# malak29/video-text-detection-system

Measured on AMD Instinct MI355X. Metric: frames/sec (detect+recognize) @720p, 1/2/4/8 MI355X; box IoU vs CPU ref, higher is better.
Workload: dtype f16

## Files before the change

### video-text-detection-system_amd/csrc/conv_halo.hip

```cpp
#include <cstdio>
#include <cstdlib>
#include "vtd_common.h"

namespace {

struct HaloParams {
    const half_t* in;
    const half_t* wgt;
    const float* bias;
    const half_t* res;
    half_t* out;
    int n, h, w, cin, cout;
    int in_hp, in_wp, in_ring, out_hp, out_wp, out_ring, res_hp, res_wp, res_ring;
    int tiles_x, tiles_y, tiles_n, relu;
    unsigned long long* stamps;
    const half_t* in2 = nullptr;
    int in2_hp = 0, in2_wp = 0, in2_c = 0, in2_ring = 0;
    int K = 0;
    int dbg;
};

template <int N>
__device__ __forceinline__ void hl_wait_vmcnt() {
    asm volatile("s_waitcnt vmcnt(%0)" ::"n"(N) : "memory");
}

template <int BN, int TW>
__global__ __launch_bounds__((BN / 64) * 256) void conv_halo_kernel(const HaloParams p) {
    constexpr int WN = BN / 64, NW = 4 * WN, NT = NW * 64, TH = 256 / TW;
    constexpr int HWD = TW + 2, HROWS = (TH + 2) * HWD, HPIECES = (HROWS + 7) / 8, HBYTES = HPIECES * 1024;
    constexpr int HPW = (HPIECES + NW - 1) / NW;
    constexpr int HPS = (HPW + 7) / 8;
    constexpr int BSTAGE = BN * 128, BPW = BN / 8 / NW;
    constexpr int EPI_ROW = BN * 4 + 16;
// ... 307 lines not shown
            if (p.res) {
#pragma unroll
                for (int e = 0; e < 4; ++e) { v0[e] += (float)rv[q][e]; v1[e] += (float)rv[q][4 + e]; }
            }
            half8 hv;
#pragma unroll
            for (int e = 0; e < 4; ++e) {
                hv[e] = (half_t)((p.relu && v0[e] < 0.f) ? 0.f : v0[e]);
                hv[4 + e] = (half_t)((p.relu && v1[e] < 0.f) ? 0.f : v1[e]);
            }
            *(half8*)(p.out + (((int64_t)img * p.out_hp + y + p.out_ring) * p.out_wp + x + p.out_ring) * p.cout + ch) = hv;
        }
    }
}

template <int TW>
int halo64_launch(const HaloParams& p, hipStream_t stream) {
    constexpr int TH = 256 / TW, HROWS = (TH + 2) * (TW + 2), HBYTES = (HROWS + 7) / 8 * 1024;
    constexpr int lds = HBYTES + 4 * 64 * 128;
    static_assert(lds >= 256 * (64 * 4 + 16) && 2 * lds <= 160 * 1024, "epilogue tile fits; two workgroups per CU");
    static bool attr_done = false;
    if (!attr_done) {
        hipError_t e = hipFuncSetAttribute((const void*)conv_halo64_kernel<TW>, hipFuncAttributeMaxDynamicSharedMemorySize, lds);
        if (e != hipSuccess) return -(int)e;
        attr_done = true;
    }
    hipLaunchKernelGGL((conv_halo64_kernel<TW>), dim3(p.n * p.tiles_y * p.tiles_x * p.tiles_n), dim3(256), lds, stream, p);
    return -(int)hipGetLastError();
}

constexpr int HS_HW = 18, HS_ROWS = 180, HS_PIECES = 23, HS_HALO_BYTES = 24 * 1024, HS_BSTAGE = 64 * 128;
constexpr int HS_LDS = HS_HALO_BYTES + 3 * HS_BSTAGE;

template <int N>
__device__ __forceinline__ void hs_wait_staged() {
    asm volatile("s_waitcnt vmcnt(%0) lgkmcnt(0)" ::"n"(N) : "memory");
}

__global__ __launch_bounds__(256, 3) void conv_halo_small_kernel(const HaloParams p) {
    constexpr int NW = 4, FN = 2, BPW = 2, HPW = 6;
    __shared__ __attribute__((aligned(16))) char smem[HS_LDS];
    char* const hb = smem;
    char* const bring = smem + HS_HALO_BYTES;

    const int nblk = gridDim.x, b = blockIdx.x;
    const int q8 = nblk >> 3, r8 = nblk & 7, xcd = b & 7;
    int tile = (xcd < r8 ? xcd * (q8 + 1) : r8 * (q8 + 1) + (xcd - r8) * q8) + (b >> 3);
    const int tn = tile % p.tiles_n;
    tile /= p.tiles_n;
    const int tx = tile % p.tiles_x;
    tile /= p.tiles_x;
    const int ty = tile % p.tiles_y;
    const int img = tile / p.tiles_y;
    const int y0 = ty * 8, x0 = tx * 16, n0 = tn * 64;

    const int tid = threadIdx.x, lane = tid & 63;
    const int w = __builtin_amdgcn_readfirstlane(tid >> 6);
    const int lrow = lane >> 3, fr = lane & 15, fq = lane >> 4;
    const int K = p.K, nchunks = p.cin >> 6;
    const bool dual = p.in2 != nullptr;

    int hoff[HPW];
#pragma unroll
    for (int k = 0; k < HPW; ++k) {
        int row = (w + k * NW) * 8 + lrow;
        row = row < HS_ROWS ? row : HS_ROWS - 1;
        const int hy = row / HS_HW, hx = row - hy * HS_HW;
        int gy = y0 - 1 + hy + p.in_ring, gx = x0 - 1 + hx + p.in_ring;
        gy = gy < p.in_hp ? gy : p.in_hp - 1;
        gx = gx < p.in_wp ? gx : p.in_wp - 1;
        hoff[k] = ((img * p.in_hp + gy) * p.in_wp + gx) * p.cin + ((lane & 7) ^ (hx & 6)) * 8;
    }
    auto issue_halo = [&](int chunk) {
#pragma unroll
        for (int k = 0; k < HPW; ++k)
            if (w + k * NW < HS_PIECES)
// ... 8 lines not shown
        }
    };
    const half_t* bsrc[BPW];
#pragma unroll
    for (int i = 0; i < BPW; ++i) {
        const int row = (i * NW + w) * 8 + lrow;
        const int chan = (row & 32) + ((row >> 2) & 3) * 8 + ((row >> 4) & 1) * 4 + (row & 3);
        bsrc[i] = p.wgt + (int64_t)(n0 + chan) * K + ((lane & 7) ^ ((row >> 1) & 7)) * 8;
    }
    auto issue_b = [&](int koff, int stage) {
#pragma unroll
        for (int i = 0; i < BPW; ++i)
            __builtin_amdgcn_global_load_lds((const VTD_AS1 void*)(bsrc[i] + koff), (VTD_AS3 void*)(bring + stage * HS_BSTAGE + (i * NW + w) * 1024), 16, 0, 0);
    };

    const int wm = w >> 1, wn = w & 1;
    const char* a_addr[3][2];
#pragma unroll
    for (int dx = 0; dx < 3; ++dx)
#pragma unroll
        for (int kk = 0; kk < 2; ++kk) a_addr[dx][kk] = hb + (wm * 4 * HS_HW + fr + dx) * 128 + (((fq + 4 * kk) ^ ((fr + dx) & 6)) << 4);
    const char* b_addr[2];
#pragma unroll
    for (int kk = 0; kk < 2; ++kk) b_addr[kk] = bring + (wn * FN * 16 + fr) * 128 + (((fq + 4 * kk) ^ ((fr >> 1) & 7)) << 4);
    floatx4 acc[FN][4];
#pragma unroll
    for (int i = 0; i < FN; ++i)
#pragma unroll
        for (int j = 0; j < 4; ++j) acc[i][j] = floatx4{0.f, 0.f, 0.f, 0.f};

    issue_halo(0);
    issue_b(0, 0);
    issue_b(p.cin, 1);
    for (int chunk = 0; chunk < nchunks; ++chunk) {
        const bool more = chunk + 1 < nchunks;
#pragma unroll
        for (int tap = 0; tap < 9; ++tap) {
            if (tap < 8 || more || dual) hs_wait_staged<BPW>(); else hs_wait_staged<0>();
            __builtin_amdgcn_s_barrier();
            const int tap2 = (tap + 2) % 9;
            const int koff2 = (tap == 7 && !more) ? 9 * p.cin : tap2 * p.cin + (chunk + (tap + 2 >= 9 ? 1 : 0)) * 64;
            if (tap < 7 || (tap == 7 && (more || dual))) issue_b(koff2, (tap + 2) % 3);
            const int row_off = ((tap / 3) * HS_HW) * 128, stage_off = (tap % 3) * HS_BSTAGE;
#pragma unroll
            for (int kk = 0; kk < 2; ++kk) {
                half8 af[4], bf[FN];
#pragma unroll
                for (int j = 0; j < 4; ++j) af[j] = *(const half8*)(a_addr[tap % 3][kk] + row_off + j * (HS_HW * 128));
#pragma unroll
                for (int i = 0; i < FN; ++i) bf[i] = *(const half8*)(b_addr[kk] + stage_off + i * 2048);
#pragma unroll
                for (int i = 0; i < FN; ++i)
#pragma unroll
                    for (int j = 0; j < 4; ++j) acc[i][j] = __builtin_amdgcn_mfma_f32_16x16x32_f16(bf[i], af[j], acc[i][j], 0, 0, 0);
            }
            if (tap == 8 && more) {
                asm volatile("s_waitcnt lgkmcnt(0)" ::: "memory");
                __builtin_amdgcn_s_barrier();
                issue_halo(chunk + 1);
                issue_b(koff2, (tap + 2) % 3);
            } else if (tap == 8 && dual) {
                asm volatile("s_waitcnt lgkmcnt(0)" ::: "memory");
                __builtin_amdgcn_s_barrier();
                issue_dual();
            }
        }
    }
    if (dual) {
        hs_wait_staged<0>();
        __builtin_amdgcn_s_barrier();
#pragma unroll
        for (int kk = 0; kk < 2; ++kk) {
            half8 af[4], bf[FN];
            const char* a2 = hb + (wm * 64 + fr) * 128 + (((fq + 4 * kk) ^ (fr & 6)) << 4);
#pragma unroll
            for (int j = 0; j < 4; ++j) af[j] = *(const half8*)(a2 + j * 2048);
#pragma unroll
            for (int i = 0; i < FN; ++i) bf[i] = *(const half8*)(b_addr[kk] + i * 2048);
#pragma unroll
            for (int i = 0; i < FN; ++i)
#pragma unroll
                for (int j = 0; j < 4; ++j) acc[i][j] = __builtin_amdgcn_mfma_f32_16x16x32_f16(bf[i], af[j], acc[i][j], 0, 0, 0);
        }
    }

    const int ch = n0 + wn * 32 + fq * 8;
    const floatx4 bias0 = *(const floatx4*)(p.bias + ch), bias1 = *(const floatx4*)(p.bias + ch + 4);
    const int x = x0 + fr;
    half8 rv[4];
    if (p.res) {
#pragma unroll
        for (int j = 0; j < 4; ++j) {
            int y = y0 + wm * 4 + j;
            y = y < p.h ? y : p.h - 1;
            const int xc = x < p.w ? x : p.w - 1;
            rv[j] = *(const half8*)(p.res + (((int64_t)img * p.res_hp + y + p.res_ring) * p.res_wp + xc + p.res_ring) * p.cout + ch);
        }
    }
#pragma unroll
    for (int j = 0; j < 4; ++j) {
        const int y = y0 + wm * 4 + j;
        if (y >= p.h || x >= p.w) continue;
        floatx4 v0 = acc[0][j] + bias0, v1 = acc[1][j] + bias1;
        if (p.res) {
#pragma unroll
            for (int e = 0; e < 4; ++e) { v0[e] += (float)rv[j][e]; v1[e] += (float)rv[j][4 + e]; }
        }
        half8 hv;
#pragma unroll
        for (int e = 0; e < 4; ++e) {
            hv[e] = (half_t)((p.relu && v0[e] < 0.f) ? 0.f : v0[e]);
            hv[4 + e] = (half_t)((p.relu && v1[e] < 0.f) ? 0.f : v1[e]);
        }
        *(half8*)(p.out + (((int64_t)img * p.out_hp + y + p.out_ring) * p.out_wp + x + p.out_ring) * p.cout + ch) = hv;
    }
}

template <int TW, bool RELU, bool RES>
__global__ __launch_bounds__(256, 1) void conv3x3_c64_persistent_kernel(const HaloParams p) {
    constexpr int TH = 256 / TW, HWD = TW + 2, HROWS = (TH + 2) * HWD, HPIECES = (HROWS + 7) / 8, HBYTES = HPIECES * 1024;
    constexpr int HPW = (HPIECES + 3) / 4;
    constexpr int WBYTES = 9 * 64 * 128;
    extern __shared__ __attribute__((aligned(16))) char smem[];
    char* const wl = smem;
    char* const hbuf = smem + WBYTES;

    const int tid = threadIdx.x, lane = tid & 63;
    const int w = __builtin_amdgcn_readfirstlane(tid >> 6);
    const int lrow = lane >> 3, fr = lane & 15, fq = lane >> 4;
    const int tiles_per_img = p.tiles_x * p.tiles_y, total = p.n * tiles_per_img;

#pragma unroll
    for (int k = 0; k < 18; ++k) {
        const int piece = w + 4 * k, tap = piece >> 3, row = (piece & 7) * 8 + lrow;
        const int c_log = (lane & 7) ^ ((row >> 1) & 7);
        const int cout = 16 * ((row & 15) >> 2) + 4 * (row >> 4) + (row & 3);
        __builtin_amdgcn_global_load_lds((const VTD_AS1 void*)(p.wgt + cout * 576 + tap * 64 + c_log * 8),
                                         (VTD_AS3 void*)(wl + piece * 1024), 16, 0, 0);
    }
    floatx4 bias4[4];
#pragma unroll
    for (int i = 0; i < 4; ++i) bias4[i] = *(const floatx4*)(p.bias + fq * 16 + i * 4);
#pragma unroll
    for (int i = 0; i < 4; ++i) asm volatile("" : "+v"(bias4[i]));

    auto tile_coords = [&](int t, int& img, int& y0, int& x0) {
        img = t / tiles_per_img;
        const int r = t - img * tiles_per_img, ty = r / p.tiles_x;
// ... 423 lines not shown
    p.relu = (c.flags & EPI_RELU) ? 1 : 0;
    p.stamps = nullptr;
    p.dbg = 0;
    if (c.in_y0 != c.in_x0 || c.in_y0 < 0 || c.K != 9 * c.in_c || c.out_c != c.cout || p.n <= 0 || (c.in_c & 63) || (c.cout & 63) ||
        (tw != 16 && tw != 32) || c.stride != 1 || c.M != p.n * c.ho * c.wo)
        return -2201;
    if ((int64_t)p.n * c.in_hp * c.in_wp * c.in_c >= (1ll << 31)) return -2202;
    const int th = 256 / tw;
    p.tiles_x = (p.w + tw - 1) / tw; p.tiles_y = (p.h + th - 1) / th; p.tiles_n = bn > 1 ? p.cout / bn : 1;
    if (bn == 2) {
        p.tiles_n = p.cout / 64;
        return tw == 16 ? halo64_launch<16>(p, stream) : halo64_launch<32>(p, stream);
    }
    if (bn == 1) {
        if (p.cin != 64 || p.cout != 64) return -2201;
        p.tiles_n = 1;
        return tw == 16 ? c64_dispatch<16>(p, stream) : c64_dispatch<32>(p, stream);
    }
    if (bn == 64 && tw == 16) return halo_launch<64, 16>(p, stream);
    if (bn == 64 && tw == 32) return halo_launch<64, 32>(p, stream);
    if (bn == 128 && tw == 16) return halo_launch<128, 16>(p, stream);
    if (bn == 128 && tw == 32) return halo_launch<128, 32>(p, stream);
    return -2201;
}

bool vtd_conv_halo_small_supported(const ConvParams& c) {
    if (!halo_common_rules(c, true) || c.ho % 8 || c.wo % 16) return false;
    if (c.in2 && (c.in2_mul != 2 || c.in2_shr != 0 || c.cin_steps2 != 1 || c.kw2 != 1 || c.seg1_steps * 64 != 9 * c.in_c || c.in2_c < 64 || (c.in2_c & 7) ||
                  c.in2_ring < 0 || 2 * (c.ho - 1) + c.in2_ring >= c.in2_hp || 2 * (c.wo - 1) + c.in2_ring >= c.in2_wp))
        return false;
    return c.in_hp >= c.ho + c.in_y0 + 2 && c.in_wp >= c.wo + c.in_y0 + 2;
}

int vtd_launch_conv_halo_small(const ConvParams& c, hipStream_t stream) {
    if (c.ho <= 0 || c.wo <= 0) return -2201;
    HaloParams p;
    p.in = c.in; p.wgt = c.wgt; p.bias = c.bias; p.res = (c.flags & EPI_RESIDUAL) ? c.res : nullptr; p.out = (half_t*)c.out;
    p.h = c.ho; p.w = c.wo; p.n = c.M / (c.ho * c.wo); p.cin = c.in_c; p.cout = c.cout;
    p.in_hp = c.in_hp; p.in_wp = c.in_wp; p.in_ring = c.in_y0 + 1;
    p.out_hp = c.out_hp; p.out_wp = c.out_wp; p.out_ring = c.out_ring;
    p.res_hp = c.res_hp; p.res_wp = c.res_wp; p.res_ring = c.res_ring;
    p.relu = (c.flags & EPI_RELU) ? 1 : 0;
    p.stamps = nullptr;
    p.dbg = 0;
    p.K = c.K;
    if (c.in2) { p.in2 = c.in2; p.in2_hp = c.in2_hp; p.in2_wp = c.in2_wp; p.in2_c = c.in2_c; p.in2_ring = c.in2_ring; }
    if (c.in_y0 != c.in_x0 || c.in_y0 < 0 || c.K != 9 * c.in_c + (c.in2 ? 64 : 0) || c.out_c != c.cout || p.n <= 0 || (c.in_c & 63) || (c.cout & 63) ||
        c.stride != 1 || c.M != p.n * c.ho * c.wo || (c.ho & 7) || (c.wo & 15) || ((c.flags & EPI_RESIDUAL) && !c.res) || c.plist)
        return -2201;
    if (c.in2 && (c.in2_mul != 2 || c.in2_shr != 0 || c.in2_c < 64 || (c.in2_c & 7) || c.in2_ring < 0 || 2 * (c.ho - 1) + c.in2_ring >= c.in2_hp ||
                  2 * (c.wo - 1) + c.in2_ring >= c.in2_wp || (int64_t)p.n * c.in2_hp * c.in2_wp * c.in2_c >= (1ll << 31)))
        return -2201;
    if (c.in_hp < c.ho + p.in_ring + 1 || c.in_wp < c.wo + p.in_ring + 1 || c.out_ring < 0 || c.out_hp < c.ho + c.out_ring || c.out_wp < c.wo + c.out_ring ||
        (p.res && (c.res_ring < 0 || c.res_hp < c.ho + c.res_ring || c.res_wp < c.wo + c.res_ring)))
        return -2201;
    if ((int64_t)p.n * c.in_hp * c.in_wp * c.in_c >= (1ll << 31)) return -2202;
    p.tiles_x = p.w / 16; p.tiles_y = p.h / 8; p.tiles_n = p.cout / 64;
    hipLaunchKernelGGL(conv_halo_small_kernel, dim3(p.n * p.tiles_y * p.tiles_x * p.tiles_n), dim3(256), 0, stream, p);
    return -(int)hipGetLastError();
}
```

### video-text-detection-system_amd/csrc/vtd_api.cpp

```cpp
#include <algorithm>
#include <cmath>
#include <cstdio>
#include <cstdlib>
#include <cstring>
#include <map>
#include <memory>
#include <string>
#include <vector>

#include "../../include/vtd.h"
#include "vtd_common.h"

int vtd_launch_conv(const ConvParams& p, int cfg, hipStream_t stream);
int vtd_conv_num_configs();
bool vtd_conv_config_valid(const ConvParams& p, int cfg);
int vtd_launch_preprocess(const uint8_t* frames, int n, int H, int W, half_t* out, const int* xb, const int* xk, int ksx,
                          const int* yb, const int* yk, int ksy, int max_rows, hipStream_t stream);
int vtd_launch_nchw_to_input(const float* x, half_t* out, int n, hipStream_t stream);
int vtd_launch_maxpool(const TensorDesc& in, const TensorDesc& out, int n, int kh, int kw, int sh, int sw, int pad_h, int pad_w,
                       hipStream_t stream);
void vtd_stem_pool_pack_weights(const float* w_folded, half_t* packed);
int vtd_launch_stem_pool(const TensorDesc& in, const TensorDesc& out, const half_t* w_packed, const float* bias, int n, hipStream_t stream);
extern "C" int vtd_head_entry_halo_steps(int py, int px, int nch1, int* out);
int vtd_launch_head_entry_halo(const ConvParams& c, const int* steps_dev, int nsteps, int big_tiles, hipStream_t stream);
#ifdef VTD_EXPERIMENTAL_CANDIDATES
extern "C" int vtd_head_entry_half_schedule(const int* steps, int nsteps, int* out);
int vtd_launch_head_entry_half(const ConvParams& c, const int* sched_dev, int nsteps, hipStream_t stream);
int vtd_head_entry_pair_tables(int py, int px, int c2ch, int* half_steps, int* plan);
int vtd_launch_head_entry_pair(const ConvParams& c, const int* half_steps_dev, const int* plan_dev, int nh, hipStream_t stream);
#endif
bool vtd_conv_halo_supported(const ConvParams& c, int* bn_out, int* tw_out);
bool vtd_conv_halo_c64_supported(const ConvParams& c, int tw);
int vtd_launch_conv_halo(const ConvParams& c, int bn, int tw, hipStream_t stream);
bool vtd_conv_halo_small_supported(const ConvParams& c);
int vtd_launch_conv_halo_small(const ConvParams& c, hipStream_t stream);
bool vtd_pointwise128_supported(const ConvParams& c);
int vtd_launch_pointwise128(const ConvParams& c, hipStream_t stream);
void vtd_head_tail_pack_w1(const half_t* w1_gemm, half_t* packed);
void vtd_head_tail_pack_w2(const float* w2, half_t* packed);
int vtd_launch_head_tail(const TensorDesc& in, const half_t* w1, const float* bias1, const half_t* w2, float b2, float* out, int n,
                         hipStream_t stream);

int vtd_launch_crop_resize(const uint8_t* frames, int H, int W, const int32_t* boxes, int ncrops, uint8_t* out, hipStream_t s);
int vtd_launch_crnn_conv1(const uint8_t* in_u8, const float* in_f32, const half_t* w, const float* bias, half_t* out, int n, hipStream_t s);
int vtd_launch_lstm(const half_t* xs, const half_t* whh, half_t* hout, int D, int T, hipStream_t s);
int vtd_launch_ctc_greedy(const float* logits, int n, int T, int V, int ld, const int32_t* id2char, int blank, int apply_softmax,
                          int32_t* out, hipStream_t s);
int vtd_launch_compact_rows(const float* in, float* out, int64_t rows, int V, int ld, hipStream_t s);
int vtd_dbloss_ws_bytes();
int vtd_launch_dbloss(const float* prob, const float* thresh, const float* prob_t, const float* thresh_t, int64_t n, float smooth, double* workspace,
                      float* out4, double* sums5, hipStream_t stream);
int vtd_launch_dbloss_backward(const float* prob, const float* thresh, const float* prob_t, const float* thresh_t, int64_t n, float smooth,
                               const double* sums5, const float* grad_out4, float* grad_prob, float* grad_thresh, hipStream_t stream);
int vtd_launch_binary_counts(const float* pred, const float* target, int64_t n, float threshold, int64_t* counts4, hipStream_t stream);
int vtd_launch_adamw(const vtd_adamw_tensor* tensors, int count, const vtd_adamw_hyper* hyper, hipStream_t stream);
int64_t vtd_dbhead_ws_bytes(int n, int H, int W, int backward);
int vtd_launch_dbhead_pack(const void* x, int dtype, int n, int H, int W, void* feats, hipStream_t s);
int vtd_launch_dbhead_forward(const void* feats, int n, int H, int W, const vtd_dbhead_params* params, int training, float momentum, float eps,
                              void* ws, float* prob, float* thresh, float* stats_out, hipStream_t s);
int vtd_launch_dbhead_backward_input(int n, int H, int W, const vtd_dbhead_params* params, void* scratch, float* dfeats, float* dscale, hipStream_t s);
int vtd_launch_dbhead_unpack_input_grad(const float* dfeats, const float* dscale, int n, int H, int W, float* out, hipStream_t s);
int64_t vtd_fpn_ws_bytes(int n, int h5, int w5, int c5, int mode);
int vtd_launch_fpn_pack_tap(const void* x, int dtype, int n, int channels, int H, int W, void* out, hipStream_t s);
int vtd_launch_fpn_unpack_p2(const void* p2, int n, int H, int W, float* out, hipStream_t s);
int vtd_launch_fpn_pack_grad(const float* g, int n, int H, int W, float* out, hipStream_t s);
int vtd_launch_fpn_forward(const void* const* taps, int n, int h5, int w5, int c5, const vtd_fpn_params* params, void* ws, void* p2_out, hipStream_t s);
int vtd_launch_fpn_backward(const void* const* taps, int n, int h5, int w5, int c5, const vtd_fpn_params* params, const void* ws, const float* dp2,
                            const float* dscale, const vtd_fpn_params* grads, void* scratch, hipStream_t s);
// ... 160 lines not shown
    std::memset(&p, 0, sizeof(p));
    p.in = c.in.ptr; p.wgt = c.w; p.k_hi_step = c.k_hi_step; p.cin_steps = c.cin_steps; p.kw = c.kw; p.s_step = c.s_step; p.r_step = c.r_step; p.bias = c.bias;
    p.res = c.has_res ? c.res.ptr : nullptr;
    p.out = (c.flags & (EPI_OUT_F32 | EPI_OUT_F16)) ? c.out_f32 : (void*)c.out.ptr;
    p.M = n * c.ho * c.wo; p.K = c.K; p.cout = c.cout; p.cout_pad = c.cout_pad;
    p.ho = c.ho; p.wo = c.wo;
    p.in_hp = c.in.hp; p.in_wp = c.in.wp; p.in_c = c.in.c; p.in_y0 = c.in_y0; p.in_x0 = c.in_x0; p.stride = c.stride;
    p.out_hp = c.out.hp; p.out_wp = c.out.wp; p.out_c = c.out.c; p.out_ring = c.out.ring;
    p.res_hp = c.res.hp; p.res_wp = c.res.wp; p.res_ring = c.res.ring; p.res_shift = c.res_shift;
    p.ps_cout = c.ps_cout; p.flags = c.flags; p.ldc = c.ldc;
    p.seg_cols = c.seg_cols;
    for (int i = 0; i < 3; ++i) { p.seg_out[i] = c.seg_out[i]; p.seg_ldc[i] = c.seg_ldc[i]; }
    p.head_w = c.head_w; p.head_b = c.head_b; p.prob_out = (float*)c.out_f32;
    if (c.plist) {
        p.plist = c.plist; p.tile_combo = c.tile_combo; p.tiles_per_img = c.tiles_per_img;
        p.plist_b = c.plist_b; p.tile_combo_b = c.tile_combo_b; p.tiles_per_img_b = c.tiles_per_img_b;
        p.in2 = c.in2.ptr; p.in2_hp = c.in2.hp; p.in2_wp = c.in2.wp; p.in2_c = c.in2.c; p.in2_ring = c.in2.ring;
        p.seg1_steps = c.seg1_steps; p.cin_steps2 = c.cin_steps2; p.kw2 = c.kw2; p.s_step2 = c.s_step2; p.r_step2 = c.r_step2;
        p.bias_tab = c.bias_tab; p.img_h = c.img_h; p.img_w = c.img_w;
        p.M = n * c.tiles_per_img * 128;
    }
    p.pool_pw = c.pool_pw;
    if (c.dual) {
        p.in2 = c.in2.ptr; p.in2_hp = c.in2.hp; p.in2_wp = c.in2.wp; p.in2_c = c.in2.c; p.in2_ring = c.in2.ring;
        p.in2_mul = c.in2_mul; p.in2_shr = c.in2_shr;
        p.seg1_steps = c.seg1_steps; p.cin_steps2 = c.cin_steps2; p.kw2 = 1; p.s_step2 = 0; p.r_step2 = 0;
    }
}

static const int kHaloCfg = 100;
static const int kHaloC64Cfg = 101;
static const int kHalo64Cfg = 104;
static const int kHaloSmallCfg = 108;
static const int kHeadEntryHalo256Cfg = 103;
static const int kHeadEntryPairCfg = 105;
static const int kPointwiseCfg = 106;
static const int kHeadEntryHalfCfg = 107;
static const int kHeadEntryHaloCfg = 102;
static bool halo_enabled() {
    const char* e = std::getenv("VTD_HALO_CONV");
    return !(e && e[0] == '0');
}

static int pick_tile_height(const ConvParams& p, int table_cfg) {
    if (const char* e = std::getenv("VTD_TILE_HEIGHT_MODEL"); e && e[0] == '0') return table_cfg;
    if (std::getenv("VTD_FORCE_CONV_CFG")) return table_cfg;
    static const struct { int cfg, bm, bn; double eff; } family[5] = {{0, 256, 128, 1.0}, {14, 256, 128, 1.04}, {13, 272, 128, 0.92}, {12, 208, 128, 0.80},
                                                                      {15, 256, 256, 1.07}};
    auto cost_of = [&](int cfg) -> double {
        for (const auto& k : family)
            if (k.cfg == cfg) {
                if (!vtd_conv_config_valid(p, k.cfg)) return 0.0;
                const int64_t tiles = (int64_t)((p.M + k.bm - 1) / k.bm) * (p.cout_pad / k.bn);
                return (double)((tiles + 255) / 256) * k.bm * k.bn / k.eff;
            }
        return 0.0;
    };
    int best = table_cfg;
    double best_cost = cost_of(table_cfg);
    if (best_cost == 0.0) return table_cfg;
    const double keep = best_cost * 0.94;
    double other_cost = keep;
    for (const auto& k : family) {
        if (k.cfg == table_cfg) continue;
        const double c = cost_of(k.cfg);
        if (c > 0.0 && c < other_cost) { other_cost = c; best = k.cfg; }
    }
    (void)best_cost;
    return best;
}

static int launch_conv_op(const ConvOp& c, int n, hipStream_t s, int cfg = -1, float* prob_out = nullptr) {
    ConvParams p;
    fill_conv_params(c, n, p);
    if (prob_out) p.prob_out = prob_out;
#ifdef VTD_EXPERIMENTAL_CANDIDATES
    if (cfg == kHeadEntryPairCfg) {
        if (!c.hp_half_steps || !c.tile_combo_border) return ERR_GEOMETRY;
        return vtd_launch_head_entry_pair(p, c.hp_half_steps, c.hp_plan, c.hp_nh, s);
    }
    if (cfg == kHeadEntryHalfCfg) {
        if (!c.hh_sched || !c.tile_combo_border) return ERR_GEOMETRY;
        return vtd_launch_head_entry_half(p, c.hh_sched, c.he_nsteps, s);
    }
#else
    if (cfg == kHeadEntryPairCfg || cfg == kHeadEntryHalfCfg) return ERR_GEOMETRY;
#endif
    if (cfg == kHeadEntryHaloCfg || cfg == kHeadEntryHalo256Cfg) {
        if (!c.he_steps || !c.tile_combo_border) return ERR_GEOMETRY;
        return vtd_launch_head_entry_halo(p, c.he_steps, c.he_nsteps, cfg == kHeadEntryHalo256Cfg ? 1 : 0, s);
    }
    if (cfg == kHaloCfg || cfg == kHaloC64Cfg || cfg == kHalo64Cfg) {
        int bn = 0, tw = 0;
        if (!vtd_conv_halo_supported(p, &bn, &tw)) return ERR_GEOMETRY;
        return vtd_launch_conv_halo(p, cfg == kHaloC64Cfg ? 1 : cfg == kHalo64Cfg ? 2 : bn, tw, s);
    }
    if (cfg == kHaloSmallCfg) return vtd_conv_halo_small_supported(p) ? vtd_launch_conv_halo_small(p, s) : ERR_GEOMETRY;
    if (cfg == kPointwiseCfg) return vtd_launch_pointwise128(p, s);
    if (!c.plist && (cfg == 0 || cfg == 12 || cfg == 13 || cfg == 14 || cfg == 15)) cfg = pick_tile_height(p, cfg);
    return vtd_launch_conv(p, cfg, s);
}

static int launch_border_tiles(const ConvOp& c, int n, hipStream_t s) {
    if (!c.tile_combo_border || c.tiles_border <= 0) return ERR_GEOMETRY;
    ConvParams pb;
    fill_conv_params(c, n, pb);
    pb.tile_combo = c.tile_combo_border; pb.tiles_per_img = c.tiles_border; pb.M = n * c.tiles_border * 128;
    pb.plist_b = nullptr; pb.tile_combo_b = nullptr; pb.tiles_per_img_b = 0;
    return vtd_launch_conv(pb, 9, s);
}

static int autotune_conv(const ConvOp& c, int n, hipStream_t s, int* best_cfg) {
    ConvParams p;
    fill_conv_params(c, n, p);
    hipEvent_t e0, e1;
    VTD_HIP_CHECK(hipEventCreate(&e0));
    VTD_HIP_CHECK(hipEventCreate(&e1));
    float best = 1e30f;
    int best_id = -1, rc = 0;
    if (p.plist) {
        const char* fc = std::getenv("VTD_FORCE_CLASSED_CFG");
        if (fc && (vtd_conv_config_valid(p, std::atoi(fc)) || ((std::atoi(fc) == kHeadEntryHaloCfg || std::atoi(fc) == kHeadEntryHalo256Cfg) && c.he_steps) ||
                   (std::atoi(fc) == kHeadEntryHalfCfg && c.hh_sched) ||
                   (std::atoi(fc) == kHeadEntryPairCfg && c.hp_half_steps))) {
            (void)hipEventDestroy(e0);
            (void)hipEventDestroy(e1);
            *best_cfg = std::atoi(fc);
            return 0;
        }
    }
// ... 34 lines not shown
        }
    }
    if (!rc && vtd_pointwise128_supported(p)) {
        if (!(rc = vtd_launch_pointwise128(p, s))) {
            (void)hipEventRecord(e0, s);
            for (int rep = 0; rep < 3 && !rc; ++rep) rc = vtd_launch_pointwise128(p, s);
            (void)hipEventRecord(e1, s);
            if (hipEventSynchronize(e1) != hipSuccess) rc = ERR_ARG;
            float ms = 0.f;
            (void)hipEventElapsedTime(&ms, e0, e1);
            if (!rc && ms < best) { best = ms; best_id = kPointwiseCfg; }
        }
    }
    int hbn = 0, htw = 0;
    const char* force = std::getenv("VTD_FORCE_HALO");
    bool pinned = false;
    if (!rc && halo_enabled() && vtd_conv_halo_supported(p, &hbn, &htw)) {
        if (force && (force[0] == '1' || force[0] == '2' || force[0] == '3')) best = 1e30f;
        for (int variant = 0; variant < 3 && !rc; ++variant) {
            if (variant == 1 && !vtd_conv_halo_c64_supported(p, htw)) continue;
            const int bn = variant == 1 ? 1 : variant == 2 ? 2 : hbn;
            if ((rc = vtd_launch_conv_halo(p, bn, htw, s))) break;
            (void)hipEventRecord(e0, s);
            for (int rep = 0; rep < 3 && !rc; ++rep) rc = vtd_launch_conv_halo(p, bn, htw, s);
            (void)hipEventRecord(e1, s);
            if (hipEventSynchronize(e1) != hipSuccess) rc = ERR_ARG;
            float ms = 0.f;
            (void)hipEventElapsedTime(&ms, e0, e1);
            const int vid = variant == 1 ? kHaloC64Cfg : variant == 2 ? kHalo64Cfg : kHaloCfg;
            const bool pin = (variant == 1 && force && force[0] == '2') || (variant == 2 && force && force[0] == '3');
            if (!rc && !pinned && (ms < best || pin)) { best = ms; best_id = vid; pinned = pin; }
        }
    }
    if (!rc && halo_enabled() && vtd_conv_halo_small_supported(p)) {
        if (!(rc = vtd_launch_conv_halo_small(p, s))) {
            (void)hipEventRecord(e0, s);
            for (int rep = 0; rep < 3 && !rc; ++rep) rc = vtd_launch_conv_halo_small(p, s);
            (void)hipEventRecord(e1, s);
            if (hipEventSynchronize(e1) != hipSuccess) rc = ERR_ARG;
            float ms = 0.f;
            (void)hipEventElapsedTime(&ms, e0, e1);
            const bool pin = force && force[0] == '4';
            if (!rc && (pin || (!pinned && ms < best))) { best = ms; best_id = kHaloSmallCfg; }
        }
    }
    (void)hipEventDestroy(e0);
    (void)hipEventDestroy(e1);
    *best_cfg = best_id;
    if (const char* v = std::getenv("VTD_AUTOTUNE_VERBOSE"); v && v[0] == '1')
        std::fprintf(stderr, "[autotune] M=%d N=%d K=%d%s -> cfg %d (%.1f us per launch)\n", p.M, p.cout, p.K, p.plist ? " classed" : "", best_id,
                     best / 3.f * 1e3f);
    return rc;
}

static bool autotune_enabled() {
    const char* e = std::getenv("VTD_AUTOTUNE");
    return !(e && e[0] == '0');
}

struct ResampleAxis {
    int ksize = 0;
    std::vector<int> bounds, kk;
};
static ResampleAxis pillow_axis(int in_size, int out_size) {
    ResampleAxis a;
    const double scale = (double)in_size / out_size;
    const double fscale = scale < 1.0 ? 1.0 : scale;
    const double support = fscale;
    a.ksize = (int)std::ceil(support) * 2 + 1;
    a.bounds.assign(2 * (size_t)out_size, 0);
    a.kk.assign((size_t)out_size * a.ksize, 0);
    std::vector<double> pre(a.ksize);
    for (int xx = 0; xx < out_size; ++xx) {
        const double center = (xx + 0.5) * scale, ss = 1.0 / fscale;
        int xmin = (int)(center - support + 0.5);
        if (xmin < 0) xmin = 0;
// ... 36 lines not shown
    int alloc_tensor(TensorDesc& t) {
        void* p = nullptr;
        int rc = arena.alloc(&p, (size_t)tensor_elems(t) * sizeof(half_t), true);
        t.ptr = (half_t*)p;
        return rc;
    }
    const std::vector<float>* get(const std::string& k, size_t numel) const {
        auto it = sd.find(k);
        if (it == sd.end() || it->second.size() != numel) return nullptr;
        return &it->second;
    }
};

static std::string conv_signature(const ConvOp& c) {
    char buf[192];
    int len = std::snprintf(buf, sizeof buf, "conv|in%dx%dx%d|out%dx%d|co%d|K%d|s%d|f%x|r%d|c%d", c.in.h, c.in.w, c.in.c, c.ho, c.wo, c.cout, c.K,
                            c.stride, (unsigned)c.flags, c.has_res ? 1 + c.res_shift : 0, c.plist ? 1 : 0);
    if (c.dual) len += std::snprintf(buf + len, sizeof buf - len, "|x%dm%ds%d", c.in2.c, c.in2_mul, c.in2_shr);
    if (c.pool_pw) std::snprintf(buf + len, sizeof buf - len, "|p2x%d", c.pool_pw);
    return buf;
}

static bool config_valid_for(const ConvOp& c, int n, int cfg) {
    ConvParams p;
    fill_conv_params(c, n, p);
    if (cfg == kHeadEntryPairCfg) return p.plist && c.hp_half_steps && c.tile_combo_border;
    if (cfg == kHeadEntryHalfCfg) return p.plist && c.hh_sched && c.tile_combo_border;
    if (cfg == kHeadEntryHaloCfg || cfg == kHeadEntryHalo256Cfg) return p.plist && c.he_steps && c.tile_combo_border;
    if (cfg == kHaloCfg || cfg == kHaloC64Cfg || cfg == kHalo64Cfg) {
        int bn = 0, tw = 0;
        if (!vtd_conv_halo_supported(p, &bn, &tw)) return false;
        return cfg != kHaloC64Cfg || vtd_conv_halo_c64_supported(p, tw);
    }
    if (cfg == kHaloSmallCfg) return vtd_conv_halo_small_supported(p);
    if (cfg == kPointwiseCfg) return vtd_pointwise128_supported(p);
    return cfg >= 0 && cfg < vtd_conv_num_configs() && vtd_conv_config_valid(p, cfg);
}

static int choose_config(ModelBase* m, const ConvOp& c, int n, hipStream_t s, int* cfg) {
    const std::string key = conv_signature(c) + "|n" + std::to_string(n);
    auto it = m->tuning.find(key);
    const bool forced = std::getenv("VTD_FORCE_CLASSED_CFG") || std::getenv("VTD_FORCE_HALO");
    if (const char* fc = std::getenv("VTD_FORCE_CONV_CFG"); fc && !c.plist && config_valid_for(c, n, std::atoi(fc))) {
        *cfg = std::atoi(fc);
        return 0;
    }
    if (const char* fp = std::getenv("VTD_FORCE_POINTWISE"); fp && fp[0] == '1' && config_valid_for(c, n, kPointwiseCfg)) {
        *cfg = kPointwiseCfg;
        return 0;
    }
    if (!forced && it != m->tuning.end() && config_valid_for(c, n, it->second)) {
        *cfg = it->second;
        return 0;
    }
    *cfg = -1;
    if (!autotune_enabled()) return 0;
    int rc = autotune_conv(c, n, s, cfg);
    if (!rc && *cfg >= 0) {
        m->tuning[key] = *cfg;
        m->tuning_measured = true;
    }
    return rc;
}

static int set_tuning_text(ModelBase* m, const char* text) {
    if (!m || !text) return ERR_ARG;
    const char* p = text;
// ... 1321 lines not shown
        for (auto& sp : d->ev_spans) {
            float ms = 0.f;
            e = hipEventElapsedTime(&ms, sp.second.first, sp.second.second);
            if (e != hipSuccess) return -(int)e;
            d->prof_ms[sp.first] += ms;
            d->prof_calls[sp.first] += 1;
        }
        d->ev_spans.clear();
        d->ev_used = 0;
    }
    const Op& o = d->ops[op_index];
    if (o.kind == Op::CONV) {
        const ConvOp& c = o.conv;
        static const char* kTile[] = {"256,128,s3", "128,128,s2", "128,128,s3", "256,64,s2", "256,64,s3", "128,64,s2", "128,64,s3",
                                      "64,256,s2", "128,64,s2,classed", "128,64,s3,classed", "256,64,s2,classed", "256,64,s3,classed", "208,128,s3", "272,128,s3", "256,128,s3,16w", "256,256,s2", "128,64,s6"};
        int cfg = -1;
        if (!d->tuned.empty()) cfg = d->tuned.rbegin()->second[op_index];
        if (cfg == kHeadEntryPairCfg)
            std::snprintf(name, name_cap, "head_entry_pair M/img=%d N=%d K=%d (lateral+smooth+head conv composed; border classes in the "
                          "next slot)", c.ho * c.wo, c.cout, c.K);
        else if (cfg == kHeadEntryHalfCfg)
            std::snprintf(name, name_cap, "head_entry_half M/img=%d N=%d K=%d (lateral+smooth+head conv composed, half halos two steps ahead; border classes in the "
                          "next slot)", c.ho * c.wo, c.cout, c.K);
        else if (cfg == kHeadEntryHalo256Cfg)
            std::snprintf(name, name_cap, "head_entry_halo256 M/img=%d N=%d K=%d (lateral+smooth+head conv composed; border classes in the "
                          "next slot)", c.ho * c.wo, c.cout, c.K);
        else if (cfg == kHeadEntryHaloCfg)
            std::snprintf(name, name_cap, "head_entry_halo M/img=%d N=%d K=%d (lateral+smooth+head conv composed; border classes in the "
                          "next slot)", c.ho * c.wo, c.cout, c.K);
        else if (cfg == kPointwiseCfg)
            std::snprintf(name, name_cap, "pointwise128 1x1%s streaming M/img=%d N=%d K=%d", c.has_res ? "+top-down add" : "", c.ho * c.wo, c.cout, c.K);
        else if (cfg == kHaloSmallCfg)
            std::snprintf(name, name_cap, "conv_halo_small 3x3 M/img=%d N=%d K=%d", c.ho * c.wo, c.cout, c.K);
        else if (cfg == kHaloCfg || cfg == kHaloC64Cfg || cfg == kHalo64Cfg)
            std::snprintf(name, name_cap, "conv_halo%s 3x3 M/img=%d N=%d K=%d", cfg == kHaloC64Cfg ? "_c64_persistent" : cfg == kHalo64Cfg ? "64" : "",
                          c.ho * c.wo, c.cout, c.K);
        else
            std::snprintf(name, name_cap, "conv_igemm<%s> M/img=%d N=%d K=%d%s", (cfg >= 0 && cfg < 17) ? kTile[cfg] : "default",
                          c.ho * c.wo, c.cout, c.K, c.plist ? " (lateral+smooth+head conv composed)" : "");
    } else if (o.kind == Op::POOL) {
        std::snprintf(name, name_cap, "maxpool %dx%d/s%d", o.pk[0], o.pk[1], o.pk[2]);
    } else if (o.kind == Op::BORDER) {
        std::snprintf(name, name_cap, "conv_igemm<128,64,s3,classed> border classes of the composed head entry (%d tiles/img)", o.conv.tiles_border);
    } else if (o.kind == Op::HEADTAIL) {
        std::snprintf(name, name_cap, "head_tail ConvT1+BN+ReLU+ConvT2+sigmoid fused M/img=%d N=256 K=64", o.conv.ho * o.conv.wo);
    } else if (o.kind == Op::STEMPOOL) {
        std::snprintf(name, name_cap, "stem_pool conv7x7/s2+BN+ReLU+maxpool3x3/s2 fused M/img=%d N=64 K=147", 320 * 320);
    } else {
        std::snprintf(name, name_cap, "conv_igemm<64,256,s2> ConvT1+ConvT2+sigmoid fused M/img=%d", o.conv.ho * o.conv.wo);
    }
    const bool have = d->prof_ms.size() == d->ops.size();
    *total_ms = have ? d->prof_ms[op_index] : 0.0;
    *calls = have ? d->prof_calls[op_index] : 0;
    *total_macs = have ? d->prof_macs[op_index] : 0.0;
    return 0;
}

int vtd_detector_read_tap(vtd_detector* d, const char* name, int n, float* host_out, int64_t capacity, vtd_stream stream) {
    if (!d || !name || !host_out) return ERR_ARG;
    if (!d->finalized) return ERR_NOT_FINALIZED;
    auto it = d->taps.find(name);
    if (it == d->taps.end()) return ERR_UNKNOWN_KEY;
    const TensorDesc& t = it->second;
    if (n <= 0 || n > t.n) return ERR_BATCH;
    const int creal = (std::string(name) == "input") ? 3 : t.c;
    if (capacity < (int64_t)n * creal * t.h * t.w) return ERR_CAPACITY;
// ... 251 lines not shown
```

Measured before the change: 12640.

## Add loader-wave variant of small halo conv and autotune against original

Adds a 320-thread variant of the small 3x3 halo convolution in which a fifth wave does all global-to-LDS DMA (halo and weight stages) while four compute waves only wait on barriers and run MFMA. The autotuner now times both variants and picks the faster per conv signature. The aim is to take DMA issue and vmcnt waits off the compute waves. In exchange it adds an extra wave per workgroup and relies on barrier-only synchronization between producer and consumers. Cycle-stamp instrumentation behind a compile flag is also added.

```diff
diff --git a/video-text-detection-system_amd/csrc/conv_halo.hip b/video-text-detection-system_amd/csrc/conv_halo.hip
--- a/video-text-detection-system_amd/csrc/conv_halo.hip
+++ b/video-text-detection-system_amd/csrc/conv_halo.hip
@@ -1,5 +1,10 @@
 #include <cstdio>
 #include <cstdlib>
+#ifdef VTD_HALO_SMALL_STAMPS
+#include <algorithm>
+#include <map>
+#include <vector>
+#endif
 #include "vtd_common.h"
 
 namespace {
@@ -373,6 +378,23 @@
 constexpr int HS_HW = 18, HS_ROWS = 180, HS_PIECES = 23, HS_HALO_BYTES = 24 * 1024, HS_BSTAGE = 64 * 128;
 constexpr int HS_LDS = HS_HALO_BYTES + 3 * HS_BSTAGE;
 
+#ifdef VTD_HALO_SMALL_STAMPS
+#define HS_STAMP_STATE unsigned long long st_acc[3] = {0, 0, 0}, st_t = __builtin_amdgcn_s_memtime(); const unsigned long long st_t0 = st_t
+#define HS_LAP(i) do { const unsigned long long st_n = __builtin_amdgcn_s_memtime(); st_acc[i] += st_n - st_t; st_t = st_n; } while (0)
+#define HS_STAMP_WRITE(nw) do { if (p.stamps && lane == 0) { unsigned long long* st_o = p.stamps + ((int64_t)blockIdx.x * (nw) + w) * 8; \
+    st_o[0] = st_acc[0]; st_o[1] = st_acc[1]; st_o[2] = st_acc[2]; st_o[3] = st_t - st_t0; \
+    st_o[4] = __builtin_amdgcn_s_getreg(4 | (31 << 11)); st_o[5] = __builtin_amdgcn_s_getreg(20 | (31 << 11)); } } while (0)
+#define HS_STAMP_ENTRY const unsigned long long st_entry = __builtin_amdgcn_s_memtime()
+#define HS_STAMP_EXIT(nw) do { if (p.stamps && lane == 0) { unsigned long long* st_o = p.stamps + ((int64_t)blockIdx.x * (nw) + w) * 8; \
+    st_o[6] = st_entry; st_o[7] = __builtin_amdgcn_s_memtime(); } } while (0)
+#else
+#define HS_STAMP_STATE
+#define HS_LAP(i)
+#define HS_STAMP_WRITE(nw)
+#define HS_STAMP_ENTRY
+#define HS_STAMP_EXIT(nw)
+#endif
+
 template <int N>
 __device__ __forceinline__ void hs_wait_staged() {
     asm volatile("s_waitcnt vmcnt(%0) lgkmcnt(0)" ::"n"(N) : "memory");
@@ -383,6 +405,7 @@
     __shared__ __attribute__((aligned(16))) char smem[HS_LDS];
     char* const hb = smem;
     char* const bring = smem + HS_HALO_BYTES;
+    HS_STAMP_ENTRY;
 
     const int nblk = gridDim.x, b = blockIdx.x;
     const int q8 = nblk >> 3, r8 = nblk & 7, xcd = b & 7;
@@ -457,15 +480,18 @@
     issue_halo(0);
     issue_b(0, 0);
     issue_b(p.cin, 1);
+    HS_STAMP_STATE;
     for (int chunk = 0; chunk < nchunks; ++chunk) {
         const bool more = chunk + 1 < nchunks;
 #pragma unroll
         for (int tap = 0; tap < 9; ++tap) {
             if (tap < 8 || more || dual) hs_wait_staged<BPW>(); else hs_wait_staged<0>();
             __builtin_amdgcn_s_barrier();
+            HS_LAP(0);
             const int tap2 = (tap + 2) % 9;
             const int koff2 = (tap == 7 && !more) ? 9 * p.cin : tap2 * p.cin + (chunk + (tap + 2 >= 9 ? 1 : 0)) * 64;
             if (tap < 7 || (tap == 7 && (more || dual))) issue_b(koff2, (tap + 2) % 3);
+            HS_LAP(1);
             const int row_off = ((tap / 3) * HS_HW) * 128, stage_off = (tap % 3) * HS_BSTAGE;
 #pragma unroll
             for (int kk = 0; kk < 2; ++kk) {
@@ -479,18 +505,24 @@
 #pragma unroll
                     for (int j = 0; j < 4; ++j) acc[i][j] = __builtin_amdgcn_mfma_f32_16x16x32_f16(bf[i], af[j], acc[i][j], 0, 0, 0);
             }
+            HS_LAP(2);
             if (tap == 8 && more) {
                 asm volatile("s_waitcnt lgkmcnt(0)" ::: "memory");
                 __builtin_amdgcn_s_barrier();
+                HS_LAP(0);
                 issue_halo(chunk + 1);
                 issue_b(koff2, (tap + 2) % 3);
+                HS_LAP(1);
             } else if (tap == 8 && dual) {
                 asm volatile("s_waitcnt lgkmcnt(0)" ::: "memory");
                 __builtin_amdgcn_s_barrier();
+                HS_LAP(0);
                 issue_dual();
-            }
-        }
-    }
+                HS_LAP(1);
+            }
+        }
+    }
+    HS_STAMP_WRITE(4);
     if (dual) {
         hs_wait_staged<0>();
         __builtin_amdgcn_s_barrier();
@@ -539,6 +571,209 @@
         }
         *(half8*)(p.out + (((int64_t)img * p.out_hp + y + p.out_ring) * p.out_wp + x + p.out_ring) * p.cout + ch) = hv;
     }
+    HS_STAMP_EXIT(4);
+}
+
+__global__ __launch_bounds__(320, 4) void conv_halo_small_lw_kernel(const HaloParams p) {
+    constexpr int NW = 4, FN = 2, BP = 8;
+    extern __shared__ __attribute__((aligned(16))) char smem[];
+    char* const hb = smem;
+    char* const bring = smem + HS_HALO_BYTES;
+    HS_STAMP_ENTRY;
+
+    const int nblk = gridDim.x, b = blockIdx.x;
+    const int q8 = nblk >> 3, r8 = nblk & 7, xcd = b & 7;
+    int tile = (xcd < r8 ? xcd * (q8 + 1) : r8 * (q8 + 1) + (xcd - r8) * q8) + (b >> 3);
+    const int tn = tile % p.tiles_n;
+    tile /= p.tiles_n;
+    const int tx = tile % p.tiles_x;
+    tile /= p.tiles_x;
+    const int ty = tile % p.tiles_y;
+    const int img = tile / p.tiles_y;
+    const int y0 = ty * 8, x0 = tx * 16, n0 = tn * 64;
+
+    const int tid = threadIdx.x, lane = tid & 63;
+    const int w = __builtin_amdgcn_readfirstlane(tid >> 6);
+    const int lrow = lane >> 3, fr = lane & 15, fq = lane >> 4;
+    const int K = p.K, nchunks = p.cin >> 6;
+    const bool dual = p.in2 != nullptr;
+
+    if (w == NW) {
+        VTD_AS3 char* const lds = (VTD_AS3 char*)smem;
+        auto dma = [](const void* base, unsigned off, VTD_AS3 char* dst) {
+            asm volatile("" : "+s"(base));
+            __builtin_amdgcn_global_load_lds((const VTD_AS1 void*)((const char*)base + off), (VTD_AS3 void*)dst, 16, 0, 0);
+        };
+        unsigned hoff[HS_PIECES];
+#pragma unroll
+        for (int k = 0; k < HS_PIECES; ++k) {
+            int row = k * 8 + lrow;
+            row = row < HS_ROWS ? row : HS_ROWS - 1;
+            const int hy = row / HS_HW, hx = row - hy * HS_HW;
+            int gy = y0 - 1 + hy + p.in_ring, gx = x0 - 1 + hx + p.in_ring;
+            gy = gy < p.in_hp ? gy : p.in_hp - 1;
+            gx = gx < p.in_wp ? gx : p.in_wp - 1;
+            hoff[k] = 2u * (unsigned)(((img * p.in_hp + gy) * p.in_wp + gx) * p.cin + ((lane & 7) ^ (hx & 6)) * 8);
+        }
+        auto issue_halo = [&](int chunk) {
+#pragma unroll
+            for (int k = 0; k < HS_PIECES; ++k) dma(p.in + chunk * 64, hoff[k], lds + k * 1024);
+        };
+        auto issue_dual = [&]() {
+            int l = lane;
+            asm volatile("" : "+v"(l));
+#pragma unroll
+            for (int k = 0; k < 16; ++k) {
+                const int row = k * 8 + (l >> 3), r = row >> 4, c = row & 15;
+                const int off = ((img * p.in2_hp + 2 * (y0 + r) + p.in2_ring) * p.in2_wp + 2 * (x0 + c) + p.in2_ring) * p.in2_c + ((l & 7) ^ (c & 6)) * 8;
+                dma(p.in2, 2u * (unsigned)off, lds + k * 1024);
+            }
+        };
+        const half_t* const wbase = p.wgt + (int64_t)n0 * K;
+        unsigned boff[BP];
+#pragma unroll
+        for (int k = 0; k < BP; ++k) {
+            const int row = k * 8 + lrow;
+            const int chan = (row & 32) + ((row >> 2) & 3) * 8 + ((row >> 4) & 1) * 4 + (row & 3);
+            boff[k] = 2u * (unsigned)(chan * K + ((lane & 7) ^ ((row >> 1) & 7)) * 8);
+        }
+        auto issue_b = [&](int koff, int stage) {
+#pragma unroll
+            for (int k = 0; k < BP; ++k) dma(wbase + koff, boff[k], lds + HS_HALO_BYTES + stage * HS_BSTAGE + k * 1024);
+        };
+
+        issue_halo(0);
+        issue_b(0, 0);
+        issue_b(p.cin, 1);
+        HS_STAMP_STATE;
+        for (int chunk = 0; chunk < nchunks; ++chunk) {
+            const bool more = chunk + 1 < nchunks;
+#pragma unroll
+            for (int tap = 0; tap < 9; ++tap) {
+                if (tap < 8 || more || dual) hl_wait_vmcnt<BP>(); else hl_wait_vmcnt<0>();
+                __builtin_amdgcn_s_barrier();
+                HS_LAP(0);
+                const int tap2 = (tap + 2) % 9;
+                const int koff2 = (tap == 7 && !more) ? 9 * p.cin : tap2 * p.cin + (chunk + (tap + 2 >= 9 ? 1 : 0)) * 64;
+                if (tap < 7 || (tap == 7 && (more || dual))) issue_b(koff2, (tap + 2) % 3);
+                if (tap == 8 && more) {
+                    HS_LAP(1);
+                    __builtin_amdgcn_s_barrier();
+                    HS_LAP(0);
+                    issue_halo(chunk + 1);
+                    issue_b(koff2, (tap + 2) % 3);
+                } else if (tap == 8 && dual) {
+                    HS_LAP(1);
+                    __builtin_amdgcn_s_barrier();
+                    HS_LAP(0);
+                    issue_dual();
+                }
+                HS_LAP(1);
+            }
+        }
+        HS_STAMP_WRITE(5);
+        if (dual) {
+            hl_wait_vmcnt<0>();
+            __builtin_amdgcn_s_barrier();
+        }
+        HS_STAMP_EXIT(5);
+        return;
+    }
+
+    const int wm = w >> 1, wn = w & 1;
+    const char* a_addr[3][2];
+#pragma unroll
+    for (int dx = 0; dx < 3; ++dx)
+#pragma unroll
+        for (int kk = 0; kk < 2; ++kk) a_addr[dx][kk] = hb + (wm * 4 * HS_HW + fr + dx) * 128 + (((fq + 4 * kk) ^ ((fr + dx) & 6)) << 4);
+    const char* b_addr[2];
+#pragma unroll
+    for (int kk = 0; kk < 2; ++kk) b_addr[kk] = bring + (wn * FN * 16 + fr) * 128 + (((fq + 4 * kk) ^ ((fr >> 1) & 7)) << 4);
+    floatx4 acc[FN][4];
+#pragma unroll
+    for (int i = 0; i < FN; ++i)
+#pragma unroll
+        for (int j = 0; j < 4; ++j) acc[i][j] = floatx4{0.f, 0.f, 0.f, 0.f};
+
+    HS_STAMP_STATE;
+    for (int chunk = 0; chunk < nchunks; ++chunk) {
+        const bool more = chunk + 1 < nchunks;
+#pragma unroll
+        for (int tap = 0; tap < 9; ++tap) {
+            asm volatile("s_waitcnt lgkmcnt(0)" ::: "memory");
+            __builtin_amdgcn_s_barrier();
+            HS_LAP(0);
+            const int row_off = ((tap / 3) * HS_HW) * 128, stage_off = (tap % 3) * HS_BSTAGE;
+#pragma unroll
+            for (int kk = 0; kk < 2; ++kk) {
+                half8 af[4], bf[FN];
+#pragma unroll
+                for (int j = 0; j < 4; ++j) af[j] = *(const half8*)(a_addr[tap % 3][kk] + row_off + j * (HS_HW * 128));
+#pragma unroll
+                for (int i = 0; i < FN; ++i) bf[i] = *(const half8*)(b_addr[kk] + stage_off + i * 2048);
+#pragma unroll
+                for (int i = 0; i < FN; ++i)
+#pragma unroll
+                    for (int j = 0; j < 4; ++j) acc[i][j] = __builtin_amdgcn_mfma_f32_16x16x32_f16(bf[i], af[j], acc[i][j], 0, 0, 0);
+            }
+            HS_LAP(2);
+            if (tap == 8 && (more || dual)) {
+                asm volatile("s_waitcnt lgkmcnt(0)" ::: "memory");
+                __builtin_amdgcn_s_barrier();
+                HS_LAP(0);
+            }
+        }
+    }
+    HS_STAMP_WRITE(5);
+    if (dual) {
+        asm volatile("s_waitcnt lgkmcnt(0)" ::: "memory");
+        __builtin_amdgcn_s_barrier();
+#pragma unroll
+        for (int kk = 0; kk < 2; ++kk) {
+            half8 af[4], bf[FN];
+            const char* a2 = hb + (wm * 64 + fr) * 128 + (((fq + 4 * kk) ^ (fr & 6)) << 4);
+#pragma unroll
+            for (int j = 0; j < 4; ++j) af[j] = *(const half8*)(a2 + j * 2048);
+#pragma unroll
+            for (int i = 0; i < FN; ++i) bf[i] = *(const half8*)(b_addr[kk] + i * 2048);
+#pragma unroll
+            for (int i = 0; i < FN; ++i)
+#pragma unroll
+                for (int j = 0; j < 4; ++j) acc[i][j] = __builtin_amdgcn_mfma_f32_16x16x32_f16(bf[i], af[j], acc[i][j], 0, 0, 0);
+        }
+    }
+
+    const int ch = n0 + wn * 32 + fq * 8;
+    const floatx4 bias0 = *(const floatx4*)(p.bias + ch), bias1 = *(const floatx4*)(p.bias + ch + 4);
+    const int x = x0 + fr;
+    half8 rv[4];
+    if (p.res) {
+#pragma unroll
+        for (int j = 0; j < 4; ++j) {
+            int y = y0 + wm * 4 + j;
+            y = y < p.h ? y : p.h - 1;
+            const int xc = x < p.w ? x : p.w - 1;
+            rv[j] = *(const half8*)(p.res + (((int64_t)img * p.res_hp + y + p.res_ring) * p.res_wp + xc + p.res_ring) * p.cout + ch);
+        }
+    }
+#pragma unroll
+    for (int j = 0; j < 4; ++j) {
+        const int y = y0 + wm * 4 + j;
+        if (y >= p.h || x >= p.w) continue;
+        floatx4 v0 = acc[0][j] + bias0, v1 = acc[1][j] + bias1;
+        if (p.res) {
+#pragma unroll
+            for (int e = 0; e < 4; ++e) { v0[e] += (float)rv[j][e]; v1[e] += (float)rv[j][4 + e]; }
+        }
+        half8 hv;
+#pragma unroll
+        for (int e = 0; e < 4; ++e) {
+            hv[e] = (half_t)((p.relu && v0[e] < 0.f) ? 0.f : v0[e]);
+            hv[4 + e] = (half_t)((p.relu && v1[e] < 0.f) ? 0.f : v1[e]);
+        }
+        *(half8*)(p.out + (((int64_t)img * p.out_hp + y + p.out_ring) * p.out_wp + x + p.out_ring) * p.cout + ch) = hv;
+    }
+    HS_STAMP_EXIT(5);
 }
 
 template <int TW, bool RELU, bool RES>
@@ -1028,7 +1263,7 @@
     return c.in_hp >= c.ho + c.in_y0 + 2 && c.in_wp >= c.wo + c.in_y0 + 2;
 }
 
-int vtd_launch_conv_halo_small(const ConvParams& c, hipStream_t stream) {
+static int halo_small_launch(const ConvParams& c, hipStream_t stream, bool lw) {
     if (c.ho <= 0 || c.wo <= 0) return -2201;
     HaloParams p;
     p.in = c.in; p.wgt = c.wgt; p.bias = c.bias; p.res = (c.flags & EPI_RESIDUAL) ? c.res : nullptr; p.out = (half_t*)c.out;
@@ -1052,6 +1287,76 @@
         return -2201;
     if ((int64_t)p.n * c.in_hp * c.in_wp * c.in_c >= (1ll << 31)) return -2202;
     p.tiles_x = p.w / 16; p.tiles_y = p.h / 8; p.tiles_n = p.cout / 64;
-    hipLaunchKernelGGL(conv_halo_small_kernel, dim3(p.n * p.tiles_y * p.tiles_x * p.tiles_n), dim3(256), 0, stream, p);
+    const int grid = p.n * p.tiles_y * p.tiles_x * p.tiles_n;
+#ifdef VTD_HALO_SMALL_STAMPS
+    static const bool want_stamps = [] { const char* e = getenv("VTD_HALO_STAMPS"); return e && e[0] == '1'; }();
+    if (want_stamps) {
+        const int nw = lw ? 5 : 4;
+        const size_t bytes = (size_t)grid * nw * 64;
+        unsigned long long* dev = nullptr;
+        if (hipMalloc(&dev, bytes) != hipSuccess) return -2204;
+        p.stamps = dev;
+        if (lw) hipLaunchKernelGGL(conv_halo_small_lw_kernel, dim3(grid), dim3(320), HS_LDS, stream, p);
+        else hipLaunchKernelGGL(conv_halo_small_kernel, dim3(grid), dim3(256), 0, stream, p);
+        (void)hipStreamSynchronize(stream);
+        unsigned long long* h = (unsigned long long*)malloc(bytes);
+        (void)hipMemcpy(h, dev, bytes, hipMemcpyDeviceToHost);
+        double sum[2][4] = {};
+        for (int i = 0; i < grid * nw; ++i)
+            for (int k = 0; k < 4; ++k) sum[i % nw == 4][k] += (double)h[8 * i + k];
+        const int steps = 9 * (p.cin >> 6) + (p.in2 ? 1 : 0);
+        for (int g = 0; g < (lw ? 2 : 1); ++g) {
+            const double cnt = (double)grid * (g ? 1 : 4);
+            fprintf(stderr, "[conv_halo_small%s stamps] K=%d res=%d grid %d %s: per wave cycles: wait+barrier %.0f  LDS-DMA issue %.0f  reads+MFMA %.0f  K loop %.0f  (%d K-steps)\n",
+                    lw ? "_lw" : "", p.K, p.res ? 1 : 0, grid, g ? "loader wave" : "waves 0-3", sum[g][0] / cnt, sum[g][1] / cnt, sum[g][2] / cnt, sum[g][3] / cnt, steps);
+        }
+        {
+            std::map<unsigned, std::vector<std::pair<unsigned long long, int>>> ev;
+            int simd_hist[5][4] = {}, same_as_w0 = 0;
+            double life = 0;
+            for (int g = 0; g < grid; ++g) {
+                const unsigned long long* o = h + (size_t)g * nw * 8;
+                const unsigned cu = (unsigned)((o[4] >> 8) & 0x7f) | ((unsigned)(o[5] & 15) << 8);
+                ev[cu].push_back({o[6], +1});
+                ev[cu].push_back({o[7], -1});
+                life += (double)(o[7] - o[6]);
+                for (int wv = 0; wv < nw; ++wv) simd_hist[wv][(o[wv * 8 + 4] >> 4) & 3]++;
+                if (lw && ((o[4 * 8 + 4] >> 4) & 3) == ((o[4] >> 4) & 3)) same_as_w0++;
+            }
+            double area = 0, span = 0;
+            int peak_sum = 0;
+            for (auto& kv : ev) {
+                auto& v = kv.second;
+                std::sort(v.begin(), v.end());
+                int cur = 0, peak = 0;
+                for (size_t i = 0; i + 1 < v.size(); ++i) {
+                    cur += v[i].second;
+                    peak = cur > peak ? cur : peak;
+                    area += (double)cur * (double)(v[i + 1].first - v[i].first);
+                }
+                span += (double)(v.back().first - v.front().first);
+                peak_sum += peak;
+            }
+            fprintf(stderr, "[conv_halo_small%s stamps] K=%d residency: %zu CUs, workgroups per CU: mean %.2f, peak %.2f; wave 0 entry to exit %.0f cycles; SIMD of wave 0..%d:",
+                    lw ? "_lw" : "", p.K, ev.size(), area / span, (double)peak_sum / ev.size(), life / grid, nw - 1);
+            for (int wv = 0; wv < nw; ++wv) fprintf(stderr, " [%d %d %d %d]", simd_hist[wv][0], simd_hist[wv][1], simd_hist[wv][2], simd_hist[wv][3]);
+            if (lw) fprintf(stderr, "; loader on wave 0's SIMD in %d of %d workgroups", same_as_w0, grid);
+            hipFuncAttributes fa{};
+            int occ = 0;
+            const void* fn = lw ? (const void*)conv_halo_small_lw_kernel : (const void*)conv_halo_small_kernel;
+            (void)hipFuncGetAttributes(&fa, fn);
+            (void)hipOccupancyMaxActiveBlocksPerMultiprocessor(&occ, fn, lw ? 320 : 256, 0);
+            fprintf(stderr, "; runtime: %d registers, %zu B LDS, %d workgroups per CU\n", fa.numRegs, fa.sharedSizeBytes, occ);
+        }
+        free(h);
+        (void)hipFree(dev);
+        return 0;
+    }
+#endif
+    if (lw) hipLaunchKernelGGL(conv_halo_small_lw_kernel, dim3(grid), dim3(320), HS_LDS, stream, p);
+    else hipLaunchKernelGGL(conv_halo_small_kernel, dim3(grid), dim3(256), 0, stream, p);
     return -(int)hipGetLastError();
 }
+
+int vtd_launch_conv_halo_small(const ConvParams& c, hipStream_t stream) { return halo_small_launch(c, stream, false); }
+int vtd_launch_conv_halo_small_lw(const ConvParams& c, hipStream_t stream) { return halo_small_launch(c, stream, true); }
diff --git a/video-text-detection-system_amd/csrc/vtd_api.cpp b/video-text-detection-system_amd/csrc/vtd_api.cpp
--- a/video-text-detection-system_amd/csrc/vtd_api.cpp
+++ b/video-text-detection-system_amd/csrc/vtd_api.cpp
@@ -34,6 +34,7 @@
 int vtd_launch_conv_halo(const ConvParams& c, int bn, int tw, hipStream_t stream);
 bool vtd_conv_halo_small_supported(const ConvParams& c);
 int vtd_launch_conv_halo_small(const ConvParams& c, hipStream_t stream);
+int vtd_launch_conv_halo_small_lw(const ConvParams& c, hipStream_t stream);
 bool vtd_pointwise128_supported(const ConvParams& c);
 int vtd_launch_pointwise128(const ConvParams& c, hipStream_t stream);
 void vtd_head_tail_pack_w1(const half_t* w1_gemm, half_t* packed);
@@ -260,6 +261,7 @@
 static const int kHaloC64Cfg = 101;
 static const int kHalo64Cfg = 104;
 static const int kHaloSmallCfg = 108;
+static const int kHaloSmallLwCfg = 109;
 static const int kHeadEntryHalo256Cfg = 103;
 static const int kHeadEntryPairCfg = 105;
 static const int kPointwiseCfg = 106;
@@ -324,6 +326,7 @@
         return vtd_launch_conv_halo(p, cfg == kHaloC64Cfg ? 1 : cfg == kHalo64Cfg ? 2 : bn, tw, s);
     }
     if (cfg == kHaloSmallCfg) return vtd_conv_halo_small_supported(p) ? vtd_launch_conv_halo_small(p, s) : ERR_GEOMETRY;
+    if (cfg == kHaloSmallLwCfg) return vtd_conv_halo_small_supported(p) ? vtd_launch_conv_halo_small_lw(p, s) : ERR_GEOMETRY;
     if (cfg == kPointwiseCfg) return vtd_launch_pointwise128(p, s);
     if (!c.plist && (cfg == 0 || cfg == 12 || cfg == 13 || cfg == 14 || cfg == 15)) cfg = pick_tile_height(p, cfg);
     return vtd_launch_conv(p, cfg, s);
@@ -424,16 +427,17 @@
             if (!rc && !pinned && (ms < best || pin)) { best = ms; best_id = vid; pinned = pin; }
         }
     }
-    if (!rc && halo_enabled() && vtd_conv_halo_small_supported(p)) {
-        if (!(rc = vtd_launch_conv_halo_small(p, s))) {
+    for (int lw = 0; lw < 2 && !rc && halo_enabled() && vtd_conv_halo_small_supported(p); ++lw) {
+        auto launch = [&]() { return lw ? vtd_launch_conv_halo_small_lw(p, s) : vtd_launch_conv_halo_small(p, s); };
+        if (!(rc = launch())) {
             (void)hipEventRecord(e0, s);
-            for (int rep = 0; rep < 3 && !rc; ++rep) rc = vtd_launch_conv_halo_small(p, s);
+            for (int rep = 0; rep < 3 && !rc; ++rep) rc = launch();
             (void)hipEventRecord(e1, s);
             if (hipEventSynchronize(e1) != hipSuccess) rc = ERR_ARG;
             float ms = 0.f;
             (void)hipEventElapsedTime(&ms, e0, e1);
-            const bool pin = force && force[0] == '4';
-            if (!rc && (pin || (!pinned && ms < best))) { best = ms; best_id = kHaloSmallCfg; }
+            const bool pin = force && force[0] == (lw ? '5' : '4');
+            if (!rc && (pin || (!pinned && ms < best))) { best = ms; best_id = lw ? kHaloSmallLwCfg : kHaloSmallCfg; pinned = pinned || pin; }
         }
     }
     (void)hipEventDestroy(e0);
@@ -536,7 +540,7 @@
         if (!vtd_conv_halo_supported(p, &bn, &tw)) return false;
         return cfg != kHaloC64Cfg || vtd_conv_halo_c64_supported(p, tw);
     }
-    if (cfg == kHaloSmallCfg) return vtd_conv_halo_small_supported(p);
+    if (cfg == kHaloSmallCfg || cfg == kHaloSmallLwCfg) return vtd_conv_halo_small_supported(p);
     if (cfg == kPointwiseCfg) return vtd_pointwise128_supported(p);
     return cfg >= 0 && cfg < vtd_conv_num_configs() && vtd_conv_config_valid(p, cfg);
 }
@@ -1924,6 +1928,8 @@
             std::snprintf(name, name_cap, "pointwise128 1x1%s streaming M/img=%d N=%d K=%d", c.has_res ? "+top-down add" : "", c.ho * c.wo, c.cout, c.K);
         else if (cfg == kHaloSmallCfg)
             std::snprintf(name, name_cap, "conv_halo_small 3x3 M/img=%d N=%d K=%d", c.ho * c.wo, c.cout, c.K);
+        else if (cfg == kHaloSmallLwCfg)
+            std::snprintf(name, name_cap, "conv_halo_small_lw 3x3 M/img=%d N=%d K=%d", c.ho * c.wo, c.cout, c.K);
         else if (cfg == kHaloCfg || cfg == kHaloC64Cfg || cfg == kHalo64Cfg)
             std::snprintf(name, name_cap, "conv_halo%s 3x3 M/img=%d N=%d K=%d", cfg == kHaloC64Cfg ? "_c64_persistent" : cfg == kHalo64Cfg ? "64" : "",
                           c.ho * c.wo, c.cout, c.K);
```

New measurement: 12670, median of 6. No clear change (+0.3%).
